# MCV-Univalle/HM-OpenCL

Measured on AMD Instinct MI355X. Metric: GSAD/s, higher is better.
Workload: dtype u8

## Files before the change

### hm-opencl_amd/csrc/hmme.hip

```cpp
#include "../../include/hmme.h"
#include "../../include/hmme_test.h"

#include <hip/hip_runtime.h>

#include <climits>
#include <cmath>
#include <cstdarg>
#include <cstdio>
#include <cstdlib>
#include <cstring>
#include <functional>
#include <string>
#include <type_traits>
#include <vector>

#include "me_kernels.hpp"

using hmme::MeJob;
using hmme::MeJob16;
using hmme::RefSet;

namespace {
constexpr int kMarginX = 128;
constexpr int kMarginY = 80;
// ... 227 lines not shown
  hipEvent_t ev = ctx->launch_ev[ctx->launch_seq++ % hmme_ctx::kLaunchEvents];
  HIP_TRY(ctx, hipEventRecord(ev, s));
  ctx->scratch_done = ev; ctx->scratch_stream = s; ctx->scratch_used = true;
  return HMME_OK;
}
int plane_wait(hmme_ctx* ctx, const hmme_plane* pl, hipStream_t s) {
  if (pl->fill_pending && pl->fill_stream != s) HIP_TRY(ctx, hipStreamWaitEvent(s, pl->filled, 0));
  return HMME_OK;
}
int plane_read_chain(hmme_ctx* ctx, const hmme_plane* pl, hipStream_t s) {
  if (pl->read_pending && pl->read_stream != s) HIP_TRY(ctx, hipStreamWaitEvent(s, pl->read_done, 0));
  return HMME_OK;
}
void plane_read_mark(hmme_ctx* ctx, const hmme_plane* pl, hipStream_t s) {
  pl->read_done = ctx->scratch_done; pl->read_stream = s; pl->read_pending = true;
}
int plane_write_wait(hmme_ctx* ctx, const hmme_plane* pl, hipStream_t s) {
  if (pl->fill_pending && pl->fill_stream != s) HIP_TRY(ctx, hipStreamWaitEvent(s, pl->filled, 0));
#ifndef HMME_TEST_NO_WAR_WAIT
  if (pl->read_pending && pl->read_stream != s) HIP_TRY(ctx, hipStreamWaitEvent(s, pl->read_done, 0));
#endif
  return HMME_OK;
}

struct Knobs { int tail_parts = 0, tail_launches = 0, frac_grid = 0; bool frac_job_table = false, trace = false; };
const Knobs& knobs() {
  static const Knobs k = [] {
    const auto num = [](const char* name) { const char* v = std::getenv(name); return v ? std::atoi(v) : 0; };
    return Knobs{num("HMME_TAIL_PARTS"), num("HMME_TAIL_LAUNCHES"), num("HMME_FRAC_GRID"), std::getenv("HMME_FRAC_JOB_TABLE") != nullptr, std::getenv("HMME_TRACE") != nullptr};
  }();
  return k;
}

RefSet one_ref(const uint8_t* base) {
  RefSet r;
  for (int i = 0; i < hmme::kMaxRefs; ++i) r.base[i] = base;
  return r;
}

int fair_prio(const hmme_ctx* ctx, int workgroups, bool whole_jobs) {
  return (whole_jobs || workgroups <= 4 * ctx->wg_slots) ? 1 : 0;
}

template <class F>
auto with_fen(int fen, F&& f) {
  return fen ? f(std::integral_constant<int, 1>{}) : f(std::integral_constant<int, 0>{});
}

template <int SPLIT>
int launch_search8(hmme_ctx* ctx, const RefSet& cur, int cur_ctus_x, const RefSet& ref, int ref_pitch, const void* d_jobs, int n_wg, int fen,
                   int16_t* d_mv, uint32_t* d_sad, unsigned long long* best, int n_seg_jobs, hipStream_t stream) {
  if (n_wg <= 0) return HMME_OK;
  return with_fen(fen, [&](auto f) -> int {
    const auto kernel = hmme::me_pk_gate(ctx->lambda_q16) ? hmme::me_search_kernel<decltype(f)::value, SPLIT, 1> : hmme::me_search_kernel<decltype(f)::value, SPLIT, 0>;
    hipLaunchKernelGGL(kernel, dim3(n_wg), dim3(hmme::kThreads), 0, stream, cur, cur_ctus_x, ref,
                       ref_pitch, d_jobs, ctx->lambda_q16, d_mv, d_sad, best, fair_prio(ctx, n_wg, SPLIT == 0), n_seg_jobs);
    HIP_TRY(ctx, hipGetLastError());
    return HMME_OK;
  });
}

int finalize_best(hmme_ctx* ctx, unsigned long long* d_best, const MeJob16* d_jobs, const int* d_first_strip, int n_jobs, int16_t* d_mv,
                  uint32_t* d_sad, hipStream_t stream);

int merge_table(hmme_ctx* ctx, int n_jobs, unsigned long long* preset, hipStream_t stream, unsigned long long** table) {
  if (preset) { *table = preset; return HMME_OK; }
  DevBuf& best = ctx->buf[kBest];
  bool moved;
  const int rc = ensure(ctx, best, sizeof(unsigned long long) * HMME_NUM_CTU_PARTS * (size_t)n_jobs,
                        n_jobs > 64 ? sizeof(unsigned long long) * HMME_NUM_CTU_PARTS * (size_t)n_jobs * 2 : 0, &moved);
  if (moved) ctx->best_clean = false;
  if (rc) return rc;
  if (!ctx->best_clean) HIP_TRY(ctx, hipMemsetAsync(best.p, 0xFF, best.cap, stream));
  ctx->best_clean = false;
  *table = best.as<unsigned long long>();
  return HMME_OK;
}

int launch_search8_split(hmme_ctx* ctx, const RefSet& cur, int cur_ctus_x, const RefSet& ref, int ref_pitch, const MeJob16* d_jobs,
                         const int* d_first_strip, int n_jobs, int n_split, int fen, int16_t* d_mv, uint32_t* d_sad,
                         hipStream_t stream, unsigned long long* preset_best = nullptr, bool finalize = true) {
  if (n_jobs <= 0) return HMME_OK;
  unsigned long long* best = nullptr;
  int rc = merge_table(ctx, n_jobs, preset_best, stream, &best);
  if (rc) return rc;
  rc = launch_search8<1>(ctx, cur, cur_ctus_x, ref, ref_pitch, d_jobs, n_jobs * n_split, fen, nullptr, nullptr, best, 0, stream);
  if (rc) return rc;
  return finalize ? finalize_best(ctx, best, d_jobs, d_first_strip, n_jobs, d_mv, d_sad, stream) : HMME_OK;
}

int launch_search8_segments(hmme_ctx* ctx, const RefSet& cur, int cur_ctus_x, const RefSet& ref, int ref_pitch, const void* d_table,
                            const int* d_first_strip, int n_jobs, int n_wg, int fen, int16_t* d_mv, uint32_t* d_sad, hipStream_t stream,
                            unsigned long long* best) {
  if (n_jobs <= 0 || n_wg <= 0) return HMME_OK;
  const int rc = launch_search8<2>(ctx, cur, cur_ctus_x, ref, ref_pitch, d_table, n_wg, fen, nullptr, nullptr, best, n_jobs, stream);
  if (rc) return rc;
  return finalize_best(ctx, best, hmme::me_seg_table_jobs(d_table, n_wg), d_first_strip, n_jobs, d_mv, d_sad, stream);
}


size_t lds_bytes16(int pdw, int strip_rows) { return lds_bytes16_c(pdw, strip_rows); }

int rows_max16(int pdw) {
  int r = 1;
  while (lds_bytes16(pdw, r + 1) <= kLdsBudget16) ++r;
  return r;
}
// ... 781 lines not shown
    pl.mode = SearchMode::kStrips16;
    pl.pdw = pick_pdw16(w);
    const int rmax = pl.strip_rows = rows_max16(pl.pdw), n_min = strips_for(pl.pdw, w);
    const int h = hmme::me_strip_rows16(w, w, rmax, n_min + 4);
    pl.n_strips = (w + h - 1) / h;
    const int lanes = (((w + 1) >> 1) + 2) / 3;
    auto strip_cost = [&](int k) {
      const int hk = (w + k - 1) / k;
      return 2.0 * ((((hk * lanes + 63) >> 6) + 3) >> 2) + 1.0;
    };
    if (tail && knobs.tail_parts != 1) {
      const int k_max = std::min(w / 4, 64);
      int k = knobs.tail_parts > 1 ? std::min(knobs.tail_parts, k_max) : plan_tail(tail, slots, pl.n_strips, k_max, strip_cost);
      if (k < pl.n_strips) k = pl.n_strips;
      if (k > pl.n_strips) { pl.tail_first = jobs - tail; pl.tail_parts = k; }
    }
    pl.n_wg16 = pl.tail_first * pl.n_strips + (jobs - pl.tail_first) * pl.tail_parts;
    pl.table_bytes = sizeof(MeJob16) * (size_t)pl.n_wg16;
  } else if (search_range > 64) {
    pl.mode = SearchMode::kTiles8;
    pl.table_bytes = sizeof(MeJob16) * (size_t)jobs * 4;
  } else {
    const int wgs = tail && knobs.tail_parts != 1 ? plan_tail8(tail, slots, w, knobs.tail_parts) : 0;
    if (wgs > 0) { pl.tail_first = jobs - tail; pl.tail_wgs = wgs; }
    const int head = pl.tail_first, n_tail = jobs - head;
    if (!n_tail) {
      pl.table_bytes = sizeof(MeJob) * (size_t)head;
    } else if (tail_one_launch(head, n_tail, knobs.tail_launches)) {
      pl.mode = SearchMode::kSegments8;
      pl.table_bytes = hmme::me_seg_table_bytes(head + wgs, jobs);
    } else {
      pl.mode = SearchMode::kHeadThenSegments8;
      pl.tail_jobs_off = (sizeof(MeJob) * (size_t)head + 255) & ~(size_t)255;
      pl.table_bytes = pl.tail_jobs_off + hmme::me_seg_table_bytes(wgs, n_tail);
    }
  }
  pl.first_strip = pl.mode != SearchMode::kWhole8;
  const size_t per_ref = n_refs > 0 ? (pl.table_bytes + n_refs - 1) / n_refs : pl.table_bytes;
  pl.table_grow = per_ref * hmme::kMaxRefs + 4096;
  return pl;
}
static FramePlan plan_launch(const hmme_ctx* ctx, const hmme_frame_params* fp, int count, int n_refs, bool force16 = false) {
  return plan_search(count * n_refs, n_refs, ctx->wg_slots, fp->search_range, fp->bit_depth > 8 || force16, knobs());
}

int hmme_test_tail_plan(int width, int height, int search_range, int n_pairs, int slots, int* out) {
  if (!out || width < 8 || height < 8 || width > 16384 || height > 16384 || search_range < 1 || search_range > 64 || n_pairs < 1 || slots < 1) return HMME_ERR_ARG;
  const FramePlan pl = plan_search(hmme_num_ctus(width, height) * n_pairs, n_pairs, slots, search_range, false, Knobs{});
  out[0] = pl.jobs; out[1] = pl.tail_first; out[2] = pl.tail_wgs; out[3] = pl.mode == SearchMode::kSegments8 ? 1 : 0;
  return HMME_OK;
}

int hmme_test_pk_gate(uint32_t lambda_q16) { return hmme::me_pk_gate(lambda_q16) ? 1 : 0; }

static int prep_jobs(hmme_ctx* ctx, const hmme_plane* cur, const hmme_frame_params* fp, const void* d_pred_q, int first, int count,
                     int n_refs, hipStream_t s, const FramePlan& pl, const void* d_center_q = nullptr) {
  const int jobs = pl.jobs, head = pl.tail_first, n_tail = jobs - head, w = cur->width, h = cur->height, sr = fp->search_range;
  bool moved;
  int rc = ensure(ctx, ctx->buf[kJobs], pl.table_bytes, pl.table_grow, &moved);
  if (moved) ctx->jobs_tag.valid = false;
  if (rc) return rc;
  if (pl.first_strip) {
    rc = ensure(ctx, ctx->buf[kFirstStrip], sizeof(int) * (size_t)jobs, sizeof(int) * (size_t)(jobs / (n_refs > 0 ? n_refs : 1) + 1) * hmme::kMaxRefs, &moved);
    if (moved) ctx->jobs_tag.valid = false;
    if (rc) return rc;
  }
  void* const d_jobs = ctx->buf[kJobs].p;
  int* const d_first_strip = ctx->buf[kFirstStrip].as<int>();
  hmme_ctx::TableTag tag;
  tag.valid = !d_pred_q && !d_center_q;
  tag.w = w; tag.h = h; tag.sr = sr; tag.first = first; tag.count = count; tag.pairs = n_refs;
  tag.bit_depth = fp->bit_depth | (pl.mode == SearchMode::kStrips16 && fp->bit_depth == 8 ? 0x100 : 0);
  tag.buf = d_jobs; tag.buf2 = pl.first_strip ? d_first_strip : nullptr; tag.stream = (void*)s;
  if (tag.same(ctx->jobs_tag)) return HMME_OK;
  ctx->jobs_tag.valid = false;
  const dim3 block(256);
  const auto grid = [](int n) { return dim3((n + 255) / 256); };
  const int16_t* pred = (const int16_t*)d_pred_q;
  switch (pl.mode) {
    case SearchMode::kTiles8:
      hipLaunchKernelGGL(hmme::me_prep_jobs_tile_kernel, grid(jobs), block, 0, s, (MeJob16*)d_jobs, d_first_strip, pred, first, count, n_refs, w, h, sr);
      break;
    case SearchMode::kStrips16:
      hipLaunchKernelGGL(hmme::me_prep_jobs16_kernel, grid(jobs), block, 0, s, (MeJob16*)d_jobs, d_first_strip, pred, first, count, n_refs, w, h, sr,
                         pl.n_strips, pl.strip_rows, pl.tail_first, pl.tail_parts, (const int16_t*)d_center_q);
      break;
    case SearchMode::kWhole8:
    case SearchMode::kSegments8:
    case SearchMode::kHeadThenSegments8: {
      const int idx0 = pl.mode == SearchMode::kSegments8 ? head : 0;
      if (head && idx0)
        hipLaunchKernelGGL(hmme::me_prep_whole_segments_kernel, grid(head), block, 0, s, d_jobs, d_first_strip, pred, first, count, n_refs, w, h, sr,
                           head + pl.tail_wgs, head);
      else if (head)
        hipLaunchKernelGGL(hmme::me_prep_jobs_kernel, grid(head), block, 0, s, (MeJob*)d_jobs, pred, first, count, n_refs, w, h, sr, 0, head, 1,
                           (uint32_t*)nullptr, (const int16_t*)nullptr);
      if (n_tail)
        hipLaunchKernelGGL(hmme::me_prep_segments_kernel, dim3(1), dim3(hmme::kSegPrepThreads), 0, s, (void*)((uint8_t*)d_jobs + pl.tail_jobs_off), d_first_strip,
                           pred, first, count, n_refs, w, h, sr, idx0 + pl.tail_wgs, head, n_tail, idx0);
      break;
    }
  }
  HIP_TRY(ctx, hipGetLastError());
  ctx->jobs_tag = tag;
  return HMME_OK;
}
// ... 2635 lines not shown
```

### hm-opencl_amd/csrc/me_kernels.hpp

```cpp
#pragma once

#include <hip/hip_runtime.h>
#include <stdint.h>

namespace hmme {

constexpr int kParts = 593;
constexpr int kPDW = 49;
constexpr int kWinRowsMax = 192;
constexpr int kIdxBits = 10;
constexpr uint32_t kInvCost = 3146751u;
constexpr int kGroups = 10;
constexpr int kIterPerTask = 4;
constexpr int kIterPerTaskSplit = 1;
static_assert(kIterPerTask == 4 && kIterPerTaskSplit <= 4, "2 iteration bits in the key; the guided schedule deals 4 / 2 / 1");
constexpr int kThreads = 256;

struct MeJob {
  int16_t ctu_x, ctu_y;
  int16_t lt_x, lt_y;
  int16_t rb_x, rb_y;
  int16_t pred_x, pred_y;
};
static_assert(sizeof(MeJob) == 16, "MeJob layout");
// ... 7 lines not shown
typedef __attribute__((address_space(3))) char lds_char_t;
typedef volatile __attribute__((address_space(3))) uint64_t lds_vu64_t;
typedef volatile __attribute__((address_space(3), aligned(4))) uint64_t lds_vu64a4_t;

__device__ __forceinline__ uint64_t me_pkadd(uint64_t a, uint64_t b) { return a + b; }
__device__ __forceinline__ uint64_t me_pksub(uint64_t a, uint64_t b) {
  return ((uint64_t)((uint32_t)(a >> 32) - (uint32_t)(b >> 32)) << 32) | (uint64_t)((uint32_t)a - (uint32_t)b);
}

#define ME_MAXKEY 0xFFFFFFFFu
#define ME_QSAD(pair, cur, acc) __builtin_amdgcn_qsad_pk_u16_u8((pair), (cur), (acc))
#define ME_KEYS(v, p, mult)                                                                                    \
  uint32_t v##_0, v##_1, v##_2, v##_3;                                                                         \
  asm volatile("v_mad_u32_u16 %0, %1, %2, %3" : "=v"(v##_0) : "v"((uint32_t)(p)), "s"(mult), "v"(c0));                   \
  asm volatile("v_mad_u32_u16 %0, %1, %2, %3 op_sel:[1,0,0,0]" : "=v"(v##_1) : "v"((uint32_t)(p)), "s"(mult), "v"(c1));   \
  asm volatile("v_mad_u32_u16 %0, %1, %2, %3" : "=v"(v##_2) : "v"((uint32_t)((p) >> 32)), "s"(mult), "v"(c2));           \
  asm volatile("v_mad_u32_u16 %0, %1, %2, %3 op_sel:[1,0,0,0]" : "=v"(v##_3) : "v"((uint32_t)((p) >> 32)), "s"(mult), "v"(c3))
#define ME_LIN(v, a, b)                                                                                         \
  uint32_t v##_0, v##_1, v##_2, v##_3;                                                                          \
  asm volatile("v_add3_u32 %0, %1, %2, %3" : "=v"(v##_0) : "v"(a##_0), "v"(b##_0), "v"(nc0));                              \
  asm volatile("v_add3_u32 %0, %1, %2, %3" : "=v"(v##_1) : "v"(a##_1), "v"(b##_1), "v"(nc1));                              \
  asm volatile("v_add3_u32 %0, %1, %2, %3" : "=v"(v##_2) : "v"(a##_2), "v"(b##_2), "v"(nc2));                              \
  asm volatile("v_add3_u32 %0, %1, %2, %3" : "=v"(v##_3) : "v"(a##_3), "v"(b##_3), "v"(nc3))
#define ME_SUB(v, a, b)                                                                                         \
  uint32_t v##_0, v##_1, v##_2, v##_3;                                                                          \
  asm volatile("v_sad_u32 %0, %1, %2, %3" : "=v"(v##_0) : "v"(a##_0), "v"(b##_0), "v"(c0));                                \
  asm volatile("v_sad_u32 %0, %1, %2, %3" : "=v"(v##_1) : "v"(a##_1), "v"(b##_1), "v"(c1));                                \
  asm volatile("v_sad_u32 %0, %1, %2, %3" : "=v"(v##_2) : "v"(a##_2), "v"(b##_2), "v"(c2));                                \
  asm volatile("v_sad_u32 %0, %1, %2, %3" : "=v"(v##_3) : "v"(a##_3), "v"(b##_3), "v"(c3))
__device__ __forceinline__ uint32_t me_min4(uint32_t a, uint32_t b, uint32_t c, uint32_t d) {
  uint32_t r;
  asm volatile("v_min3_u32 %0, %1, %2, %3\n\tv_min_u32 %0, %0, %4" : "=&v"(r) : "v"(a), "v"(b), "v"(c), "v"(d));
  return r;
}
#define ME_MIN4(k) me_min4(k##_0, k##_1, k##_2, k##_3)
#define ME_SUBMIN4(r, a, b)                                                                                     \
  uint32_t r;                                                                                                   \
  {                                                                                                             \
    uint32_t r##_t, r##_u;                                                                                      \
    asm volatile("v_sad_u32 %0, %3, %7, %11\n\tv_sad_u32 %1, %4, %8, %12\n\tv_sad_u32 %2, %5, %9, %13\n\t"            \
                 "v_min3_u32 %0, %0, %1, %2\n\tv_sad_u32 %1, %6, %10, %14\n\tv_min_u32 %0, %0, %1"                    \
                 : "=&v"(r), "=&v"(r##_t), "=&v"(r##_u)                                                        \
                 : "v"(a##_0), "v"(a##_1), "v"(a##_2), "v"(a##_3), "v"(b##_0), "v"(b##_1), "v"(b##_2), "v"(b##_3), "v"(c0), "v"(c1),     \
                   "v"(c2), "v"(c3));                                                                           \
  }

constexpr uint32_t kPkSlotMax = 64 * 255;
constexpr uint32_t kPkMarker = 0xFFFFu - kPkSlotMax;
constexpr uint32_t kPkMaxBits = 2 * 37;
__host__ __device__ inline bool me_pk_gate(uint32_t lambda_q16) {
  const uint64_t prod = (uint64_t)lambda_q16 * kPkMaxBits;
  return prod <= 0xFFFFFFFFull && (prod >> 16) + kPkSlotMax < kPkMarker;
}
#define ME_PKMIN(r, p)                                                                                          \
  uint32_t r;                                                                                                   \
  {                                                                                                             \
    const uint64_t r##_q = (p) + pkm;                                                                           \
    asm volatile("v_pk_min_u16 %0, %1, %2\n\tv_pk_min_u16 %0, %0, %0 op_sel:[0,1] op_sel_hi:[1,0]\n\t"                \
                 "v_mad_u32_u16 %0, %0, %3, %4"                                                                 \
                 : "=&v"(r) : "v"((uint32_t)r##_q), "v"((uint32_t)(r##_q >> 32)), "s"(mult_a), "v"(ctag));      \
  }

#define ME_MERGE_DPP_MASKED(NAME, PAD, CTRL, MASK0)                                                          \
  __device__ __forceinline__ uint32_t NAME(uint32_t a, uint32_t b) {                                         \
    uint32_t r;                                                                                              \
    asm volatile(PAD "v_min_u32_dpp %0, %2, %2 " CTRL " row_mask:0xf bank_mask:0xf\n\t"                     \
        "v_min_u32_dpp %0, %1, %1 " CTRL " row_mask:0xf bank_mask:" MASK0                                    \
        : "=&v"(r) : "v"(a), "v"(b));                                                                        \
    return r;                                                                                                \
  }
ME_MERGE_DPP_MASKED(me_merge0, "s_nop 1\n\t", "row_ror:8", "0x3")
ME_MERGE_DPP_MASKED(me_merge1, "s_nop 1\n\t", "row_half_mirror", "0x5")
ME_MERGE_DPP_MASKED(me_merge0_nn, "", "row_ror:8", "0x3")
ME_MERGE_DPP_MASKED(me_merge1_nn, "", "row_half_mirror", "0x5")
__device__ __forceinline__ uint32_t me_merge2(uint32_t a, uint32_t b) {
  u32x2_t r = __builtin_amdgcn_permlane32_swap(a, b, false, false);
  return min(r.x, r.y);
}
__device__ __forceinline__ uint32_t me_merge3(uint32_t a, uint32_t b) {
  u32x2_t r = __builtin_amdgcn_permlane16_swap(a, b, false, false);
  return min(r.x, r.y);
}
template <int DPP_CTRL>
__device__ __forceinline__ uint32_t me_merge_dpp(uint32_t a, uint32_t b, bool role) {
  const uint32_t keep = role ? b : a;
  const uint32_t give = role ? a : b;
  return min(keep, (uint32_t)__builtin_amdgcn_update_dpp(0, (int)give, DPP_CTRL, 0xf, 0xf, false));
}
#define me_merge4(a, b, role) me_merge_dpp<0x4E>(a, b, role)
#define me_merge5(a, b, role) me_merge_dpp<0xB1>(a, b, role)

__device__ __forceinline__ uint32_t me_component_bits(int v) {
  const uint32_t t = (v <= 0) ? ((uint32_t)(-v) << 1) + 1u : ((uint32_t)v << 1);
  return 2u * (31u - (uint32_t)__builtin_clz(t)) + 1u;
}
__device__ __forceinline__ uint32_t me_mv_cost(uint32_t lambda_q16, int x, int y, int pred_x, int pred_y) {
  return (lambda_q16 * (me_component_bits((x << 2) - pred_x) + me_component_bits((y << 2) - pred_y))) >> 16;
}

__device__ __forceinline__ bool me_pk_slot(int s, int& x, int& y, int& w, int& h) {
  if (s < 128) { x = (s & 7) * 8; y = (s >> 4) * 8 + ((s >> 3) & 1) * 4; w = 8; h = 4; return true; }
  if (s < 256) { x = ((s >> 1) & 7) * 8 + (s & 1) * 4; y = ((s - 128) >> 4) * 8; w = 4; h = 8; return true; }
  if (s >= 384 && s < 448) { x = (s & 7) * 8; y = ((s - 384) >> 3) * 8; w = 8; h = 8; return true; }
  return false;
}
template <int RW, int RH>
__device__ __forceinline__ void me_pk_sads(const uint32_t* wrow, int pdw, const uint8_t* __restrict__ crow, uint32_t sad[4]) {
  constexpr int ND = RW / 4;
  uint32_t c[RH][ND], d[RH][ND + 1];
#pragma unroll
  for (int r = 0; r < RH; ++r) {
#pragma unroll
    for (int k = 0; k < ND; ++k) c[r][k] = *(const uint32_t*)(crow + r * 64 + 4 * k);
#pragma unroll
    for (int k = 0; k <= ND; ++k) d[r][k] = wrow[r * pdw + k];
  }
#pragma unroll
  for (int r = 0; r < RH; ++r)
#pragma unroll
    for (int k = 0; k < ND; ++k) {
      sad[0] = __builtin_amdgcn_sad_u8(d[r][k], c[r][k], sad[0]);
#pragma unroll
      for (int j = 1; j < 4; ++j) sad[j] = __builtin_amdgcn_sad_u8(__builtin_amdgcn_alignbyte(d[r][k + 1], d[r][k], (uint32_t)j), c[r][k], sad[j]);
    }
}
__device__ __forceinline__ unsigned long long me_pk_recover(unsigned long long v, int s, const uint32_t* win, int pdw, const uint8_t* __restrict__ cur_blk,
                                                            const MeJob& job, int wx, uint32_t lambda_q16) {
  int rx, ry, rw, rh;
  if (v == ~0ull || !me_pk_slot(s, rx, ry, rw, rh)) return v;
  const int xq = (int)(v & 0xffff), y = (int)((v >> 16) & 0xffff);
  const uint32_t cost = (uint32_t)(v >> 32);
  const uint32_t* wrow = win + (y + ry) * pdw + ((xq + rx) >> 2);
  const uint8_t* crow = cur_blk + ry * 64 + rx;
  uint32_t sad[4] = {0u, 0u, 0u, 0u};
  if (rh == 4) me_pk_sads<8, 4>(wrow, pdw, crow, sad);
  else if (rw == 4) me_pk_sads<4, 8>(wrow, pdw, crow, sad);
  else me_pk_sads<8, 8>(wrow, pdw, crow, sad);
  const uint32_t by = me_component_bits(((job.lt_y + y) << 2) - job.pred_y);
#pragma unroll
  for (int j = 0; j < 4; ++j)
    if (xq + j < wx && sad[j] + ((lambda_q16 * (me_component_bits(((job.lt_x + xq + j) << 2) - job.pred_x) + by)) >> 16) == cost) return v + (unsigned long long)j;
  return v;
}

constexpr int kIdxBits16 = 8;
constexpr uint32_t kInvCost16 = 8000000u;
constexpr int kThreads16 = 256;

struct MeJob16 {
  MeJob j;
  int16_t y0, y1;
  int32_t job;
};

__host__ __device__ inline int me_xcd_unit(int p, int n) {
  const int x = p & 7, base = n >> 3, rem = n & 7;
  return x * base + (x < rem ? x : rem) + (p >> 3);
}
__host__ __device__ inline int me_xcd_position(int q, int n) {
  const int base = n >> 3, rem = n & 7, big = rem * (base + 1);
  if (q < big) return (q % (base + 1)) * 8 + q / (base + 1);
  const int r = q - big;
  return (r % base) * 8 + rem + r / base;
}

__host__ __device__ inline bool me_fold(int quads, int wy) { return (quads & 32) && (quads & 31) && (wy & 1); }
__host__ __device__ inline int me_num_tasks(int wx, int wy, int iter_per_task = kIterPerTaskSplit) {
  const int quads = (wx + 3) >> 2;
  const int wy_low = me_fold(quads, wy) ? wy - 1 : wy;
  int n = 0;
  for (int k = 5; k >= 0; --k)
    if (quads & (1 << k)) n += (((k == 5 ? wy : wy_low) + (64 >> k) - 1) / (64 >> k) + iter_per_task - 1) / iter_per_task;
  return n;
}
static_assert(sizeof(MeJob16) == 24, "MeJob16 layout");

constexpr int kGuidedT4 = 8, kGuidedT2 = 2;
__host__ __device__ inline void me_guided(int iters, int& n4, int& n2, int& n1) {
  n4 = iters > kGuidedT4 ? (iters - kGuidedT4 + 3) >> 2 : 0;
  const int rem = iters - 4 * n4;
  n2 = rem > kGuidedT2 ? (rem - kGuidedT2 + 1) >> 1 : 0;
  n1 = rem - 2 * n2;
}
__host__ __device__ inline int me_num_tasks_guided(int wx, int wy) {
  const int quads = (wx + 3) >> 2;
  const int wy_low = me_fold(quads, wy) ? wy - 1 : wy;
  int n = 0;
  for (int k = 5; k >= 0; --k)
    if (quads & (1 << k)) {
      int n4, n2, n1;
      me_guided(((k == 5 ? wy : wy_low) + (64 >> k) - 1) / (64 >> k), n4, n2, n1);
      n += n4 + n2 + n1;
    }
  return n;
// ... 27 lines not shown
    uint32_t lo[U], hi[U];
#pragma unroll
    for (int u = 0; u < U; ++u) {
      const int i = min(i0 + u * THREADS, n - 1);
      const int r = i / PDW, k = i - r * PDW;
      lo[u] = src_al[(long)r * pitch_dw + k];
      hi[u] = src_al[(long)r * pitch_dw + k + 1];
    }
#pragma unroll
    for (int u = 0; u < U; ++u) {
      const int i = i0 + u * THREADS;
      if (i < n) win[i] = __builtin_amdgcn_alignbyte(hi[u], lo[u], mis);
    }
  }
}

constexpr int kSegUnit = 4;
__host__ __device__ inline size_t me_seg_table_bytes(int n_wg, int n_jobs) { return sizeof(int4) * (size_t)n_wg + sizeof(MeJob16) * (size_t)n_jobs + sizeof(int) * ((size_t)n_jobs + 1); }
__host__ __device__ inline const int4* me_seg_table_segs(const void* t) { return (const int4*)t; }
__host__ __device__ inline const MeJob16* me_seg_table_jobs(const void* t, int n_wg) { return (const MeJob16*)((const int4*)t + n_wg); }
__host__ __device__ inline const int* me_seg_table_prefix(const void* t, int n_wg, int n_jobs) { return (const int*)(me_seg_table_jobs(t, n_wg) + n_jobs); }

constexpr int kTileStep = 129, kTileJobMask = 0x1fffffff;
template <int FEN, int SPLIT, int PK>
__global__ void __launch_bounds__(kThreads, 2)
me_search_kernel(const RefSet curs, int cur_ctus_x, const RefSet refs, int ref_pitch,
                 const void* __restrict__ jobs_v, uint32_t lambda_q16, int16_t* __restrict__ out_mv,
                 uint32_t* __restrict__ out_sad, unsigned long long* __restrict__ g_best, int fair_prio, int n_seg_jobs) {
  __shared__ uint32_t win[kWinRowsMax * kPDW];
  __shared__ unsigned long long best64[kParts];
  __shared__ int task_ctr;

  const int tid = threadIdx.x;
  const int lane = tid & 63;
#ifdef ME_SEARCH_T_TIMELINE
  const unsigned long long tl_start = wall_clock64();
#endif
  MeJob job;
  int t_first = 0, t_end = 0x7fffffff, out_job = blockIdx.x;
  unsigned long long tile_off = 0;
  int seg_j = 0, seg_g = 0, seg_end = 0, seg_head = 0;
  if constexpr (SPLIT == 2) {
    const int4 sg = me_seg_table_segs(jobs_v)[blockIdx.x];
    seg_j = sg.x; seg_g = sg.y; seg_end = sg.z; seg_head = sg.w;
    if (seg_head >= 0 && seg_g >= seg_end) return;
  } else if constexpr (SPLIT == 1) {
    const MeJob16 jb = ((const MeJob16*)jobs_v)[blockIdx.x];
    job = jb.j; t_first = jb.y0; t_end = jb.y1; out_job = jb.job & kTileJobMask;
    tile_off = (unsigned long long)(((jb.job >> 29) & 1) * kTileStep) << 16 | (unsigned long long)(((jb.job >> 30) & 1) * kTileStep);
  } else {
    job = ((const MeJob*)jobs_v)[blockIdx.x];
    out_job = me_xcd_unit(blockIdx.x, gridDim.x);
  }
#pragma unroll 1
  for (bool first_job = true;; first_job = false) {
  if constexpr (SPLIT == 2) {
    job = me_seg_table_jobs(jobs_v, gridDim.x)[seg_j].j;
    out_job = seg_j;
    if (seg_head >= 0) {
      const int* prefix = me_seg_table_prefix(jobs_v, gridDim.x, n_seg_jobs) - seg_head;
      const int p0 = prefix[seg_j], p1 = prefix[seg_j + 1];
      t_first = (seg_g - p0) * kSegUnit; t_end = (min(seg_end, p1) - p0) * kSegUnit;
      seg_g = p1; ++seg_j;
    }
    if (!first_job) __syncthreads();
  }
  if (fair_prio) __builtin_amdgcn_s_setprio(3);
  const uint8_t* __restrict__ ref_base = refs.base[job.ctu_x & 63];
  const uint8_t* __restrict__ cur_base = curs.base[job.ctu_x & 63];
  job.ctu_x &= ~63;
  const int wx = job.rb_x - job.lt_x + 1, wy = job.rb_y - job.lt_y + 1;

  for (int s = tid; s < kParts; s += kThreads) best64[s] = ~0ull;
  if (tid == 0) task_ctr = t_first;

  const uintptr_t cur_addr = (uintptr_t)(cur_base + ((long)(job.ctu_y >> 6) * cur_ctus_x + (job.ctu_x >> 6)) * kBlkBytes8);
  const uint64_t curc = (uint64_t)(uint32_t)__builtin_amdgcn_readfirstlane((uint32_t)cur_addr) |
                        (uint64_t)(uint32_t)__builtin_amdgcn_readfirstlane((uint32_t)(cur_addr >> 32)) << 32;
  if (tid < 64) me_prefetch_cur<1>(curc);
  {
    const uint8_t* src = ref_base + (long)(job.ctu_y + job.lt_y) * ref_pitch + (job.ctu_x + job.lt_x);
    const uint32_t mis = (uint32_t)(uintptr_t)src & 3u;
    const uint32_t* src_al = (const uint32_t*)(src - mis);
    const int pitch_dw = ref_pitch >> 2;
    const int n = (wy + 63) * kPDW;
    me_stage_window<kPDW, kThreads>(win, src_al, pitch_dw, n, mis, tid);
  }
  __syncthreads();
#ifdef ME_SEARCH_T_TIMELINE
  const unsigned long long tl_staged = wall_clock64();
#endif

  const int quads = (wx + 3) >> 2;
  constexpr int kIt = SPLIT ? kIterPerTaskSplit : kIterPerTask;
  constexpr bool kGuided = !SPLIT;
  const int n_tasks = kGuided ? me_num_tasks_guided(wx, wy) : min(me_num_tasks(wx, wy, kIt), t_end);
  const bool fold = me_fold(quads, wy);
  const int wy_low = fold ? wy - 1 : wy;

  const uint32_t mult_a = 1u << kIdxBits;
  const uint32_t mult_e = FEN ? (2u << kIdxBits) : (1u << kIdxBits);
  const bool rb1 = lane & 2, rb0 = lane & 1;
  int prio_quarter = 0x0fffffff;
  if (fair_prio) {
    if constexpr (!SPLIT) {
      int total = 0;
// ... 18 lines not shown
          want = min(4, max(1, (left + 3) >> 2));
          t = atomicAdd(&task_ctr, want);
        }
        t = __builtin_amdgcn_readfirstlane(t);
        want = __builtin_amdgcn_readfirstlane(want);
        if (t >= n_tasks) break;
        grab_next = t; grab_end = min(t + want, n_tasks);
      }
      t = grab_next;
    } else {
      if (lane == 0) t = atomicAdd(&task_ctr, 1);
      t = __builtin_amdgcn_readfirstlane(t);
      if (t >= n_tasks) break;
    }
    if (prio_state < 4 && (prio_state & 3) < 3) {
      prio_state += (prio_quarter << 2) + 1;
      if ((prio_state & 3) == 1) __builtin_amdgcn_s_setprio(2);
      else if ((prio_state & 3) == 2) __builtin_amdgcn_s_setprio(1);
      else __builtin_amdgcn_s_setprio(0);
    }
    int x0 = 0, k = 0, it0 = 0, n_it = 0;
    {
      int xq = 0, rem = t;
      for (int kk = 5; kk >= 0; --kk) {
        if (!(quads & (1 << kk))) continue;
        const int iters = ((kk == 5 ? wy : wy_low) + (64 >> kk) - 1) / (64 >> kk);
        int nt;
        if constexpr (kGuided) {
          int n4, n2, n1;
          me_guided(iters, n4, n2, n1);
          nt = n4 + n2 + n1;
          if (rem < nt) {
            x0 = xq * 4; k = kk;
            if (rem < n4) { it0 = 4 * rem; n_it = 4; }
            else if (rem < n4 + n2) { it0 = 4 * n4 + 2 * (rem - n4); n_it = 2; }
            else { it0 = 4 * n4 + 2 * n2 + (rem - n4 - n2); n_it = 1; }
            break;
          }
        } else {
          nt = (iters + kIt - 1) / kIt;
          if (rem < nt) {
            x0 = xq * 4; k = kk; it0 = rem * kIt; n_it = min(kIt, iters - it0);
            if constexpr (SPLIT == 2) { n_it = min(grab_end - grab_next, iters - it0); grab_next += n_it; }
            break;
          }
        }
        rem -= nt;
        xq += 1 << kk;
      }
    }
    const int ty = 64 >> k;
    const int lx = lane & ((1 << k) - 1), ly = lane >> k;
    const bool fold_part = fold && k == 5;

    uint32_t b0 = ME_MAXKEY, b1 = ME_MAXKEY, b2 = ME_MAXKEY, b3 = ME_MAXKEY, b4 = ME_MAXKEY, b5 = ME_MAXKEY,
             b6 = ME_MAXKEY, b7 = ME_MAXKEY, b8 = ME_MAXKEY, b9 = ME_MAXKEY;

    prio_state -= n_it << 2;
    for (int it = 0; it < n_it; ++it) {
      int cx = x0 + 4 * lx, cy = (it0 + it) * ty + ly;
      if (fold_part && cy == wy) { cx += 128; cy = wy - 1; }
      const bool vy = cy < wy;
      const int mvy = job.lt_y + cy, mvx = job.lt_x + cx;
      const uint32_t by = me_component_bits((mvy << 2) - job.pred_y);
      uint32_t lane_now = (uint32_t)lane;
      asm("" : "+v"(lane_now));
      const uint32_t tag = ((uint32_t)it << 8) | (lane_now << 2);
      uint32_t cc[4];
#pragma unroll
      for (int j = 0; j < 4; ++j) {
        const uint32_t cost = (lambda_q16 * (me_component_bits(((mvx + j) << 2) - job.pred_x) + by)) >> 16;
        cc[j] = (((vy && (cx + j) < wx) ? cost : kInvCost) << kIdxBits) | tag | (uint32_t)j;
      }
      const uint32_t c0 = cc[0], c1 = cc[1], c2 = cc[2], c3 = cc[3];
      const uint32_t nc0 = 0u - c0, nc1 = 0u - c1, nc2 = 0u - c2, nc3 = 0u - c3;
      uint64_t pkm = 0;
      uint32_t ctag = 0;
      if constexpr (PK) {
        const uint32_t m0 = cc[0] < (kInvCost << kIdxBits) ? cc[0] >> kIdxBits : kPkMarker, m1 = cc[1] < (kInvCost << kIdxBits) ? cc[1] >> kIdxBits : kPkMarker;
        const uint32_t m2 = cc[2] < (kInvCost << kIdxBits) ? cc[2] >> kIdxBits : kPkMarker, m3 = cc[3] < (kInvCost << kIdxBits) ? cc[3] >> kIdxBits : kPkMarker;
        pkm = (uint64_t)(m0 | m1 << 16) | (uint64_t)(m2 | m3 << 16) << 32;
        ctag = ((vy && cx < wx) ? 0u : kInvCost << kIdxBits) | tag;
      }
      const lds_char_t* lpc = (const lds_char_t*)(win + min(cy, wy - 1) * kPDW + (min(cx, wx - 1) >> 2));
#define ME8_CUR(row, q)                                                                                                            \
  ({                                                                                                                               \
    uint64_t w_;                                                                                                                   \
    asm volatile("s_load_dwordx2 %0, %1, %2" : "=s"(w_) : "s"(curc), "n"((row) * 64 + 8 * (q)));                                    \
    w_;                                                                                                                            \
  })
#define ME8_CUR_WAIT(w0, w1, w2, w3, w4, w5, w6, w7, d0, d1, d2, d3, d4, d5, d6, d7, d8, d9, d10, d11, d12, d13, d14, d15)           \
  asm volatile("" : : "v"(d0), "v"(d1), "v"(d2), "v"(d3), "v"(d4), "v"(d5), "v"(d6), "v"(d7), "v"(d8), "v"(d9), "v"(d10), "v"(d11),  \
               "v"(d12), "v"(d13), "v"(d14), "v"(d15));                                                                             \
  asm volatile("s_waitcnt lgkmcnt(0)" : "+s"(w0), "+s"(w1), "+s"(w2), "+s"(w3), "+s"(w4), "+s"(w5), "+s"(w6), "+s"(w7))
      if constexpr (PK) {
        if constexpr (FEN) {
#include "me_tree_pk_fen1.inc"
        } else {
#include "me_tree_pk_fen0.inc"
        }
      } else if constexpr (FEN) {
#include "me_tree_fen1.inc"
      } else {
#include "me_tree_fen0.inc"
      }
    }

#define ME_FLUSH(g, key_)                                                                                          \
    {                                                                                                              \
      const int slot = ME_SLOT_OF[g][lane];                                                                        \
      const uint32_t key = (key_);                                                                                 \
      const uint32_t cost = key >> kIdxBits;                                                                       \
      if (slot >= 0 && cost < kInvCost) {                                                                          \
        const int kit = (key >> 8) & 3, kl = (key >> 2) & 63, kj = key & 3;                                        \
        int bx = x0 + 4 * (kl & ((1 << k) - 1)) + kj;                                                              \
        int byy = (it0 + kit) * ty + (kl >> k);                                                                    \
        if (fold_part && byy == wy) { bx += 128; byy = wy - 1; }                                                   \
        atomicMin(&best64[slot],                                                                                   \
                  ((unsigned long long)cost << 32) | ((unsigned long long)byy << 16) | (unsigned long long)bx);    \
      }                                                                                                            \
    }
    ME_FLUSH(0, b0) ME_FLUSH(1, b1) ME_FLUSH(2, b2) ME_FLUSH(3, b3) ME_FLUSH(4, b4)
    ME_FLUSH(5, b5) ME_FLUSH(6, b6) ME_FLUSH(7, b7) ME_FLUSH(8, b8) ME_FLUSH(9, b9)
#undef ME_FLUSH
  }
#ifdef ME_SEARCH_T_TIMELINE
  const unsigned long long tl_dry = wall_clock64();
#endif
  __syncthreads();
#ifdef ME_SEARCH_T_TIMELINE
  const unsigned long long tl_all = wall_clock64();
#endif

  if constexpr (SPLIT) {
    for (int s = tid; s < kParts; s += kThreads) {
      unsigned long long v = best64[s];
      if constexpr (PK) v = me_pk_recover(v, s, win, kPDW, (const uint8_t*)cur_addr, job, wx, lambda_q16);
      if (v != ~0ull) atomicMin(&g_best[(long)out_job * kParts + s], v + tile_off);
    }
    if constexpr (SPLIT == 2) {
      if (seg_g < seg_end) continue;
    }
    return;
  }
  for (int s = tid; s < kParts; s += kThreads) {
    unsigned long long v = best64[s];
    if constexpr (PK) v = me_pk_recover(v, s, win, kPDW, (const uint8_t*)cur_addr, job, wx, lambda_q16);
    const int mvx = job.lt_x + (int)(v & 0xffff), mvy = job.lt_y + (int)((v >> 16) & 0xffff);
    const uint32_t cost = (uint32_t)(v >> 32);
    const long o = (long)out_job * kParts + s;
    out_mv[2 * o] = (int16_t)mvx;
    out_mv[2 * o + 1] = (int16_t)mvy;
    out_sad[o] = cost - me_mv_cost(lambda_q16, mvx, mvy, job.pred_x, job.pred_y);
  }
#ifdef ME_SEARCH_T_TIMELINE
  __syncthreads();
  if (lane == 0) {
    uint32_t* o = out_sad + (long)out_job * kParts;
    const int wv = tid >> 6;
    if (wv == 0) {
      const unsigned long long t1 = wall_clock64();
      uint32_t hw_id;
      asm volatile("s_getreg_b32 %0, hwreg(HW_REG_HW_ID)" : "=s"(hw_id));
      uint32_t xcc_id;
      asm volatile("s_getreg_b32 %0, hwreg(HW_REG_XCC_ID)" : "=s"(xcc_id));
      o[0] = (uint32_t)tl_start; o[1] = (uint32_t)(tl_start >> 32); o[2] = (uint32_t)(tl_staged - tl_start); o[3] = (uint32_t)(tl_all - tl_start);
      o[4] = (uint32_t)(t1 - tl_start); o[5] = hw_id; o[6] = xcc_id; o[7] = blockIdx.x;
    }
    o[8 + wv] = (uint32_t)(tl_dry - tl_start);
  }
#endif
  break;
  }
}


__host__ __device__ inline void clip_mv_q(int& x, int& y, int cu_x, int cu_y, int pic_w, int pic_h) {
  const int hor_max = (pic_w + 8 - cu_x - 1) << 2, hor_min = (-64 - 8 - cu_x + 1) << 2;
  const int ver_max = (pic_h + 8 - cu_y - 1) << 2, ver_min = (-64 - 8 - cu_y + 1) << 2;
  x = (int16_t)(x > hor_max ? hor_max : (x < hor_min ? hor_min : x));
  y = (int16_t)(y > ver_max ? ver_max : (y < ver_min ? ver_min : y));
}
__host__ __device__ inline void set_search_range(int pred_x, int pred_y, int sr, int cu_x, int cu_y, int pic_w,
                                                 int pic_h, int& lt_x, int& lt_y, int& rb_x, int& rb_y) {
  int px = pred_x, py = pred_y;
  clip_mv_q(px, py, cu_x, cu_y, pic_w, pic_h);
  int ltx = (int16_t)(px - (sr << 2)), lty = (int16_t)(py - (sr << 2));
  int rbx = (int16_t)(px + (sr << 2)), rby = (int16_t)(py + (sr << 2));
  clip_mv_q(ltx, lty, cu_x, cu_y, pic_w, pic_h);
  clip_mv_q(rbx, rby, cu_x, cu_y, pic_w, pic_h);
  lt_x = ltx >> 2; lt_y = lty >> 2; rb_x = rbx >> 2; rb_y = rby >> 2;
}

__host__ __device__ __forceinline__ MeJob me_picture_job(int i, const int16_t* __restrict__ pred_q, const int16_t* __restrict__ center_q,
                                                         int ctu_first, int ctu_count, int pic_w, int pic_h, int sr) {
  const int r = i / ctu_count;
  const int ctus_x = (pic_w + 63) >> 6, n_ctu = ctus_x * ((pic_h + 63) >> 6);
  const int ctu = ctu_first + (i - r * ctu_count);
  const int cu_x = (ctu % ctus_x) * 64, cu_y = (ctu / ctus_x) * 64;
  const long pq = 2 * ((long)r * n_ctu + ctu);
// ... 2314 lines not shown
```

### hm-opencl_amd/hmme/api.py

```python
import ctypes as C
import os
import subprocess

import numpy as np

HERE = os.path.dirname(os.path.abspath(__file__))
CSRC = os.path.join(os.path.dirname(HERE), "csrc")
LIB_PATH = os.environ.get("HMME_LIB", os.path.join(CSRC, "libhmme.so"))
NUM_PARTS = 593

SYMBOLS = ["hmme_create", "hmme_destroy", "hmme_last_error", "hmme_device_info", "hmme_set_lambda",
           "hmme_set_lambda_q16", "hmme_get_lambda_q16", "hmme_params_ocl_compat", "hmme_set_search_range",
           "hmme_slot_index", "hmme_slot_rect", "hmme_slot_index_amp_off", "hmme_amp_off_slot", "hmme_compact_amp_off", "hmme_search_ctu", "hmme_search_ctu_w", "hmme_search_refine_ctu_w", "hmme_refine_ctu_w", "hmme_search_refine_ctu", "hmme_refine_ctu", "hmme_plane_create", "hmme_plane_create_ex", "hmme_plane_bit_depth", "hmme_plane_destroy", "hmme_plane_upload_pel",
           "hmme_plane_upload_u8", "hmme_host_register", "hmme_host_unregister", "hmme_plane_set_device_u8", "hmme_plane_width", "hmme_plane_height",
           "hmme_num_ctus", "hmme_search_frame", "hmme_search_frame_device", "hmme_search_frame_multi",
           "hmme_search_frame_multi_device", "hmme_refine_frame", "hmme_refine_frame_multi_device",
           "hmme_search_pairs_device", "hmme_refine_pairs_device", "hmme_plane_upload_async",
           "hmme_upload_status", "hmme_abi_version", "hmme_build_id", "hmme_device_index", "hmme_set_error_printing",
           "hmme_weight_check", "hmme_search_pairs_w_device", "hmme_refine_pairs_w_device", "hmme_search_frame_w", "hmme_refine_frame_w",
           "hmme_bipred_check", "hmme_predict_pairs_device", "hmme_predict_frame", "hmme_search_pairs_bi_device", "hmme_refine_pairs_bi_device",
           "hmme_search_frame_bi", "hmme_refine_frame_bi",
           "hmme_bipred_weight_check", "hmme_predict_pairs_w_device", "hmme_predict_frame_w", "hmme_search_pairs_bi_w_device",
           "hmme_refine_pairs_bi_w_device", "hmme_search_frame_bi_w", "hmme_refine_frame_bi_w",
           "hmme_slot_key", "hmme_select_check", "hmme_select_pairs_device", "hmme_select_frame",
           "hmme_ref_idx_bits", "hmme_select_refs_check", "hmme_select_refs_device", "hmme_select_refs_frame",
           "hmme_predict_refs_device", "hmme_predict_refs_frame",
           "hmme_select_dirs_check", "hmme_select_dirs_device", "hmme_select_dirs_frame", "hmme_predict_bi_device", "hmme_predict_bi_frame",
           "hmme_predict_bi_weight_check", "hmme_predict_bi_w_device", "hmme_predict_bi_w_frame", "hmme_predict_refs_w_device", "hmme_predict_refs_w_frame",
           "hmme_plane_stats", "hmme_wp_estimate", "hmme_wp_estimate_420",
           "hmme_predict_chroma_pairs_device", "hmme_predict_chroma_frame", "hmme_predict_chroma_refs_device", "hmme_predict_chroma_refs_frame",
           "hmme_predict_chroma_bi_device", "hmme_predict_chroma_bi_frame",
           "hmme_residual_pairs_device", "hmme_residual_frame",
           "hmme_search_frame_bi_refs_device", "hmme_refine_frame_bi_refs_device", "hmme_search_frame_bi_refs", "hmme_refine_frame_bi_refs",
           "hmme_select_dirs_refs_check", "hmme_select_dirs_refs_device", "hmme_select_dirs_refs_frame",
           "hmme_predict_bi_refs_device", "hmme_predict_bi_refs_frame",
           "hmme_bipred_refs_weight_check", "hmme_search_frame_bi_refs_w_device", "hmme_refine_frame_bi_refs_w_device", "hmme_search_frame_bi_refs_w",
           "hmme_refine_frame_bi_refs_w",
           "hmme_predict_bi_refs_weight_check", "hmme_predict_bi_refs_w_device", "hmme_predict_bi_refs_w_frame",
           "hmme_predict_chroma_bi_refs_device", "hmme_predict_chroma_bi_refs_frame"]
TEST_SYMBOLS = ["hmme_test_time_search_kernel", "hmme_test_device_address", "hmme_test_frac_deal", "hmme_test_tail_plan", "hmme_test_stage_layout", "hmme_test_picture_job", "hmme_test_time_weight_passes", "hmme_test_time_bipred_origin",
                "hmme_test_time_wp_estimate_passes", "hmme_test_pk_gate"]
ABI_VERSION = 6


class HmmeError(RuntimeError):
    pass


class SearchParams(C.Structure):
    _fields_ = [("lt_x", C.c_int), ("lt_y", C.c_int), ("rb_x", C.c_int), ("rb_y", C.c_int),
                ("pred_x", C.c_int), ("pred_y", C.c_int), ("fen", C.c_int), ("bit_depth", C.c_int),
                ("shift_free", C.c_int)]


class Weight(C.Structure):
    _fields_ = [("w0", C.c_int), ("offset", C.c_int), ("shift", C.c_int), ("round", C.c_int)]


class WpInfo(C.Structure):
    _fields_ = [("cur_dc_sum", C.c_int64), ("cur_ac", C.c_int64), ("ref_dc_sum", C.c_int64), ("ref_ac", C.c_int64),
                ("sad_wp", C.c_int64), ("sad_nowp", C.c_int64),
                ("log2_denom", C.c_int), ("weight", C.c_int), ("offset", C.c_int), ("present", C.c_int),
                ("served_search", C.c_int), ("served_refine", C.c_int)]

    def as_dict(self):
        return {k: int(getattr(self, k)) for k, _ in self._fields_}


class SelectParams(C.Structure):
    _fields_ = [("mv_per_ctu", C.c_int), ("mv_unit", C.c_int), ("price_mv", C.c_int), ("part_mask", C.c_uint),
                ("min_depth", C.c_int), ("max_depth", C.c_int), ("cu_cost", C.c_uint32), ("pu_cost", C.c_uint32)]

    def __init__(self, mv_per_ctu=64, mv_unit=0, price_mv=0, part_mask=0xF7, min_depth=0, max_depth=3, cu_cost=0, pu_cost=0):
        super().__init__(int(mv_per_ctu), int(mv_unit), int(price_mv), int(part_mask), int(min_depth), int(max_depth), int(cu_cost), int(pu_cost))


class DirParams(C.Structure):
    _fields_ = [("dir_bits", C.c_uint32 * 3), ("list_bits", C.c_uint32 * 2)]

    def __init__(self, dir_bits=(0, 0, 0), list_bits=(0, 0)):
        super().__init__((C.c_uint32 * 3)(*[int(v) for v in dir_bits]), (C.c_uint32 * 2)(*[int(v) for v in list_bits]))


class DirRefsParams(C.Structure):
    _fields_ = [("dir_bits", C.c_uint32 * 3), ("n_refs", C.c_int * 2), ("ref_bits", (C.c_uint32 * 8) * 2), ("l1_valid_mask", C.c_uint32)]

    def __init__(self, dir_bits=(0, 0, 0), n_refs=(1, 1), ref_bits=((), ()), l1_valid_mask=None):
        rb = ((C.c_uint32 * 8) * 2)()
        for l in range(2):
            for r, v in enumerate(ref_bits[l]):
                rb[l][r] = int(v)
        mask = (1 << int(n_refs[1])) - 1 if l1_valid_mask is None else int(l1_valid_mask)
        super().__init__((C.c_uint32 * 3)(*[int(v) for v in dir_bits]), (C.c_int * 2)(*[int(v) for v in n_refs]), rb, mask)

# ... 1118 lines not shown
```

Measured before the change: 3721.

## Add packed marker-free tree body for FEN=1 with wide-slot SAD recovery

```diff
diff --git a/hm-opencl_amd/csrc/hmme.hip b/hm-opencl_amd/csrc/hmme.hip
--- a/hm-opencl_amd/csrc/hmme.hip
+++ b/hm-opencl_amd/csrc/hmme.hip
@@ -303,7 +303,12 @@
                    int16_t* d_mv, uint32_t* d_sad, unsigned long long* best, int n_seg_jobs, hipStream_t stream) {
   if (n_wg <= 0) return HMME_OK;
   return with_fen(fen, [&](auto f) -> int {
-    const auto kernel = hmme::me_pk_gate(ctx->lambda_q16) ? hmme::me_search_kernel<decltype(f)::value, SPLIT, 1> : hmme::me_search_kernel<decltype(f)::value, SPLIT, 0>;
+    constexpr int FEN = decltype(f)::value;
+    const int body = hmme::me_pk_body(ctx->lambda_q16, FEN);
+    auto kernel = body ? hmme::me_search_kernel<FEN, SPLIT, 1> : hmme::me_search_kernel<FEN, SPLIT, 0>;
+    if constexpr (FEN == 1) {
+      if (body == 2) kernel = hmme::me_search_kernel<1, SPLIT, 2>;
+    }
     hipLaunchKernelGGL(kernel, dim3(n_wg), dim3(hmme::kThreads), 0, stream, cur, cur_ctus_x, ref,
                        ref_pitch, d_jobs, ctx->lambda_q16, d_mv, d_sad, best, fair_prio(ctx, n_wg, SPLIT == 0), n_seg_jobs);
     HIP_TRY(ctx, hipGetLastError());
@@ -1191,6 +1196,8 @@
 }
 
 int hmme_test_pk_gate(uint32_t lambda_q16) { return hmme::me_pk_gate(lambda_q16) ? 1 : 0; }
+int hmme_test_pk_body(uint32_t lambda_q16, int fen) { return hmme::me_pk_body(lambda_q16, fen ? 1 : 0); }
+int hmme_test_pk_task_marker_free(int wx, int wy, int k, int it0, int n_it) { return hmme::me_task_marker_free(wx, wy, k, it0, n_it) ? 1 : 0; }
 
 static int prep_jobs(hmme_ctx* ctx, const hmme_plane* cur, const hmme_frame_params* fp, const void* d_pred_q, int first, int count,
                      int n_refs, hipStream_t s, const FramePlan& pl, const void* d_center_q = nullptr) {
diff --git a/hm-opencl_amd/csrc/me_kernels.hpp b/hm-opencl_amd/csrc/me_kernels.hpp
--- a/hm-opencl_amd/csrc/me_kernels.hpp
+++ b/hm-opencl_amd/csrc/me_kernels.hpp
@@ -83,10 +83,27 @@
   const uint64_t prod = (uint64_t)lambda_q16 * kPkMaxBits;
   return prod <= 0xFFFFFFFFull && (prod >> 16) + kPkSlotMax < kPkMarker;
 }
-#define ME_PKMIN(r, p)                                                                                          \
+constexpr uint32_t kPk2SlotMax = 16 * 12 * 255;
+__host__ __device__ inline bool me_pk2_gate(uint32_t lambda_q16) {
+  const uint64_t prod = (uint64_t)lambda_q16 * kPkMaxBits;
+  return prod <= 0xFFFFFFFFull && (prod >> 16) + kPk2SlotMax <= 0xFFFFu;
+}
+__host__ __device__ inline int me_pk_body(uint32_t lambda_q16, int fen) {
+  return (fen && me_pk2_gate(lambda_q16)) ? 2 : me_pk_gate(lambda_q16) ? 1 : 0;
+}
+__host__ __device__ inline bool me_task_marker_free(int wx, int wy, int k, int it0, int n_it) {
+  if (!(wx & 3)) return true;
+  const int quads = (wx + 3) >> 2;
+  if ((quads & -quads) == (1 << k)) return false;
+  const bool fold = (quads & 32) && (quads & 31) && (wy & 1);
+  return !(fold && k == 5 && 2 * (it0 + n_it) > wy);
+}
+#define ME_PKMIN(r, p) ME_PKMIN_Q(r, (p) + pkm)
+#define ME_PKMINE(r, p) ME_PKMIN_Q(r, ((p) << 1) + pkm)
+#define ME_PKMIN_Q(r, q)                                                                                        \
   uint32_t r;                                                                                                   \
   {                                                                                                             \
-    const uint64_t r##_q = (p) + pkm;                                                                           \
+    const uint64_t r##_q = (q);                                                                                 \
     asm volatile("v_pk_min_u16 %0, %1, %2\n\tv_pk_min_u16 %0, %0, %0 op_sel:[0,1] op_sel_hi:[1,0]\n\t"                \
                  "v_mad_u32_u16 %0, %0, %3, %4"                                                                 \
                  : "=&v"(r) : "v"((uint32_t)r##_q), "v"((uint32_t)(r##_q >> 32)), "s"(mult_a), "v"(ctag));      \
@@ -129,48 +146,74 @@
   return (lambda_q16 * (me_component_bits((x << 2) - pred_x) + me_component_bits((y << 2) - pred_y))) >> 16;
 }
 
-__device__ __forceinline__ bool me_pk_slot(int s, int& x, int& y, int& w, int& h) {
+__device__ __forceinline__ bool me_pk_slot(int s, bool wide, int& x, int& y, int& w, int& h) {
   if (s < 128) { x = (s & 7) * 8; y = (s >> 4) * 8 + ((s >> 3) & 1) * 4; w = 8; h = 4; return true; }
   if (s < 256) { x = ((s >> 1) & 7) * 8 + (s & 1) * 4; y = ((s - 128) >> 4) * 8; w = 4; h = 8; return true; }
   if (s >= 384 && s < 448) { x = (s & 7) * 8; y = ((s - 384) >> 3) * 8; w = 8; h = 8; return true; }
+  if (!wide) return false;
+  if (s < 384) {
+    const int kk = (s - 256) >> 4;
+    x = (s & 3) * 16; y = ((s >> 2) & 3) * 16; w = 16; h = 16;
+    if (kk < 4) { h = kk < 2 ? 4 : 12; if (kk & 1) y += 16 - h; }
+    else { w = kk < 6 ? 4 : 12; if (kk & 1) x += 16 - w; }
+    return true;
+  }
+  if (s < 480) { x = (s & 3) * 16; y = ((s - 448) >> 3) * 16 + ((s >> 2) & 1) * 8; w = 16; h = 8; return true; }
+  if (s < 512) { x = ((s >> 1) & 3) * 16 + (s & 1) * 8; y = ((s - 480) >> 3) * 16; w = 8; h = 16; return true; }
   return false;
 }
-template <int RW, int RH>
+template <int RW, int NR, int STEP>
 __device__ __forceinline__ void me_pk_sads(const uint32_t* wrow, int pdw, const uint8_t* __restrict__ crow, uint32_t sad[4]) {
   constexpr int ND = RW / 4;
-  uint32_t c[RH][ND], d[RH][ND + 1];
-#pragma unroll
-  for (int r = 0; r < RH; ++r) {
-#pragma unroll
-    for (int k = 0; k < ND; ++k) c[r][k] = *(const uint32_t*)(crow + r * 64 + 4 * k);
-#pragma unroll
-    for (int k = 0; k <= ND; ++k) d[r][k] = wrow[r * pdw + k];
-  }
-#pragma unroll
-  for (int r = 0; r < RH; ++r)
-#pragma unroll
-    for (int k = 0; k < ND; ++k) {
-      sad[0] = __builtin_amdgcn_sad_u8(d[r][k], c[r][k], sad[0]);
-#pragma unroll
-      for (int j = 1; j < 4; ++j) sad[j] = __builtin_amdgcn_sad_u8(__builtin_amdgcn_alignbyte(d[r][k + 1], d[r][k], (uint32_t)j), c[r][k], sad[j]);
-    }
-}
+  static_assert(RW * NR * 255 <= 0xFFFF, "the four sums are packed u16");
+  typedef uint64_t __attribute__((aligned(4))) u64a4_t;
+  uint32_t c[NR][ND];
+  uint64_t d[NR][ND];
+#pragma unroll
+  for (int r = 0; r < NR; ++r) {
+#pragma unroll
+    for (int k = 0; k < ND; ++k) c[r][k] = *(const uint32_t*)(crow + r * STEP * 64 + 4 * k);
+#pragma unroll
+    for (int k = 0; k < ND; ++k) d[r][k] = *(const u64a4_t*)(wrow + r * STEP * pdw + k);
+  }
+  uint64_t acc = 0;
+#pragma unroll
+  for (int r = 0; r < NR; ++r)
+#pragma unroll
+    for (int k = 0; k < ND; ++k) acc = ME_QSAD(d[r][k], c[r][k], acc);
+#pragma unroll
+  for (int j = 0; j < 4; ++j) sad[j] = (uint32_t)(acc >> (16 * j)) & 0xFFFFu;
+}
+template <bool WIDE>
 __device__ __forceinline__ unsigned long long me_pk_recover(unsigned long long v, int s, const uint32_t* win, int pdw, const uint8_t* __restrict__ cur_blk,
                                                             const MeJob& job, int wx, uint32_t lambda_q16) {
   int rx, ry, rw, rh;
-  if (v == ~0ull || !me_pk_slot(s, rx, ry, rw, rh)) return v;
-  const int xq = (int)(v & 0xffff), y = (int)((v >> 16) & 0xffff);
+  if (v == ~0ull || !me_pk_slot(s, WIDE, rx, ry, rw, rh)) return v;
+  const int xq = (int)(v & 0xfffc), y = (int)((v >> 16) & 0xffff);
   const uint32_t cost = (uint32_t)(v >> 32);
   const uint32_t* wrow = win + (y + ry) * pdw + ((xq + rx) >> 2);
   const uint8_t* crow = cur_blk + ry * 64 + rx;
   uint32_t sad[4] = {0u, 0u, 0u, 0u};
-  if (rh == 4) me_pk_sads<8, 4>(wrow, pdw, crow, sad);
-  else if (rw == 4) me_pk_sads<4, 8>(wrow, pdw, crow, sad);
-  else me_pk_sads<8, 8>(wrow, pdw, crow, sad);
+  int sh = 0;
+  if (!WIDE || max(rw, rh) <= 8) {
+    if (rh == 4) me_pk_sads<8, 4, 1>(wrow, pdw, crow, sad);
+    else if (rw == 4) me_pk_sads<4, 8, 1>(wrow, pdw, crow, sad);
+    else me_pk_sads<8, 8, 1>(wrow, pdw, crow, sad);
+  } else if (rh <= 8) {
+    if (rh == 4) me_pk_sads<16, 4, 1>(wrow, pdw, crow, sad);
+    else me_pk_sads<16, 8, 1>(wrow, pdw, crow, sad);
+  } else {
+    sh = 1;
+    if (rh == 12) me_pk_sads<16, 6, 2>(wrow, pdw, crow, sad);
+    else if (rw == 4) me_pk_sads<4, 8, 2>(wrow, pdw, crow, sad);
+    else if (rw == 8) me_pk_sads<8, 8, 2>(wrow, pdw, crow, sad);
+    else me_pk_sads<12, 8, 2>(wrow, pdw, crow, sad);
+  }
   const uint32_t by = me_component_bits(((job.lt_y + y) << 2) - job.pred_y);
+  v &= ~3ull;
 #pragma unroll
   for (int j = 0; j < 4; ++j)
-    if (xq + j < wx && sad[j] + ((lambda_q16 * (me_component_bits(((job.lt_x + xq + j) << 2) - job.pred_x) + by)) >> 16) == cost) return v + (unsigned long long)j;
+    if (xq + j < wx && (sad[j] << sh) + ((lambda_q16 * (me_component_bits(((job.lt_x + xq + j) << 2) - job.pred_x) + by)) >> 16) == cost) return v + (unsigned long long)j;
   return v;
 }
 
@@ -304,6 +347,7 @@
     job = ((const MeJob*)jobs_v)[blockIdx.x];
     out_job = me_xcd_unit(blockIdx.x, gridDim.x);
   }
+  if constexpr (PK == 2) asm volatile("s_waitcnt lgkmcnt(0)" ::: "memory");
 #pragma unroll 1
   for (bool first_job = true;; first_job = false) {
   if constexpr (SPLIT == 2) {
@@ -428,6 +472,7 @@
     const int ty = 64 >> k;
     const int lx = lane & ((1 << k) - 1), ly = lane >> k;
     const bool fold_part = fold && k == 5;
+    const bool marker_free = PK == 2 && me_task_marker_free(wx, wy, k, it0, n_it);
 
     uint32_t b0 = ME_MAXKEY, b1 = ME_MAXKEY, b2 = ME_MAXKEY, b3 = ME_MAXKEY, b4 = ME_MAXKEY, b5 = ME_MAXKEY,
              b6 = ME_MAXKEY, b7 = ME_MAXKEY, b8 = ME_MAXKEY, b9 = ME_MAXKEY;
@@ -469,7 +514,14 @@
   asm volatile("" : : "v"(d0), "v"(d1), "v"(d2), "v"(d3), "v"(d4), "v"(d5), "v"(d6), "v"(d7), "v"(d8), "v"(d9), "v"(d10), "v"(d11),  \
                "v"(d12), "v"(d13), "v"(d14), "v"(d15));                                                                             \
   asm volatile("s_waitcnt lgkmcnt(0)" : "+s"(w0), "+s"(w1), "+s"(w2), "+s"(w3), "+s"(w4), "+s"(w5), "+s"(w6), "+s"(w7))
-      if constexpr (PK) {
+      if constexpr (PK == 2) {
+        static_assert(PK != 2 || FEN == 1, "the marker-free body exists for FEN 1");
+        if (marker_free) {
+#include "me_tree_pk2_fen1.inc"
+        } else {
+#include "me_tree_pk_fen1.inc"
+        }
+      } else if constexpr (PK) {
         if constexpr (FEN) {
 #include "me_tree_pk_fen1.inc"
         } else {
@@ -511,7 +563,7 @@
   if constexpr (SPLIT) {
     for (int s = tid; s < kParts; s += kThreads) {
       unsigned long long v = best64[s];
-      if constexpr (PK) v = me_pk_recover(v, s, win, kPDW, (const uint8_t*)cur_addr, job, wx, lambda_q16);
+      if constexpr (PK) v = me_pk_recover<PK == 2>(v, s, win, kPDW, (const uint8_t*)cur_addr, job, wx, lambda_q16);
       if (v != ~0ull) atomicMin(&g_best[(long)out_job * kParts + s], v + tile_off);
     }
     if constexpr (SPLIT == 2) {
@@ -521,7 +573,7 @@
   }
   for (int s = tid; s < kParts; s += kThreads) {
     unsigned long long v = best64[s];
-    if constexpr (PK) v = me_pk_recover(v, s, win, kPDW, (const uint8_t*)cur_addr, job, wx, lambda_q16);
+    if constexpr (PK) v = me_pk_recover<PK == 2>(v, s, win, kPDW, (const uint8_t*)cur_addr, job, wx, lambda_q16);
     const int mvx = job.lt_x + (int)(v & 0xffff), mvy = job.lt_y + (int)((v >> 16) & 0xffff);
     const uint32_t cost = (uint32_t)(v >> 32);
     const long o = (long)out_job * kParts + s;
diff --git a/hm-opencl_amd/hmme/api.py b/hm-opencl_amd/hmme/api.py
--- a/hm-opencl_amd/hmme/api.py
+++ b/hm-opencl_amd/hmme/api.py
@@ -39,7 +39,7 @@
            "hmme_predict_bi_refs_weight_check", "hmme_predict_bi_refs_w_device", "hmme_predict_bi_refs_w_frame",
            "hmme_predict_chroma_bi_refs_device", "hmme_predict_chroma_bi_refs_frame"]
 TEST_SYMBOLS = ["hmme_test_time_search_kernel", "hmme_test_device_address", "hmme_test_frac_deal", "hmme_test_tail_plan", "hmme_test_stage_layout", "hmme_test_picture_job", "hmme_test_time_weight_passes", "hmme_test_time_bipred_origin",
-                "hmme_test_time_wp_estimate_passes", "hmme_test_pk_gate"]
+                "hmme_test_time_wp_estimate_passes", "hmme_test_pk_gate", "hmme_test_pk_body", "hmme_test_pk_task_marker_free"]
 ABI_VERSION = 6
 
 
```

After: 3778 (median of 6 runs). 1.5% higher.
